# lovelyqian/Embodied-One-Shot-Video-Recognition

Hardware: AMD Instinct MI355X
Metric: clips/sec/GPU (224², 8-seg) + 5-way-1-shot episode acc vs reference (higher is better)
Workload: dtype f32

## Files before the change

embodied-one-shot-video-recognition_amd/csrc/conv_wino_f32.hip:

```cpp
#include <type_traits>

#include "common.h"

namespace eosv {

typedef float f32x4 __attribute__((ext_vector_type(4)));
typedef float f32x16 __attribute__((ext_vector_type(16)));
typedef unsigned u32x4 __attribute__((ext_vector_type(4)));

namespace {
constexpr int WT = 64;
constexpr int WC = 64;
constexpr int WK = 8;
constexpr int IMG = 16 * WK * 64;
constexpr unsigned OOB = 0xffffff00u;
}

template <bool WIDE>
__global__ __launch_bounds__(512) void conv_wino_f32_kernel(WinoArgs a) {
  __shared__ __attribute__((aligned(16))) float smem[5 * IMG];

  const int tid = threadIdx.x;
  const int lane = tid & 63;
  const int wid = __builtin_amdgcn_readfirstlane(tid >> 6);
  const int H = a.H, W = a.W, C = a.C;
  const int TH = (H + 1) >> 1, TW = (W + 1) >> 1, TT = TH * TW;
  const long long T = (long long)a.N * TT;
  const int ncb = C / WC;
  const int nmt = (int)((T + WT - 1) / WT);
  const int nb = nmt * ncb, G = gridDim.x;
  const float* __restrict__ x = a.x;

  auto tile_of = [&](long long t, int& n, int& th, int& tw) {
    int rem;
    if (WIDE) {
      n = (int)(t / TT);
      rem = (int)(t - (long long)n * TT);
    } else {
      n = wino_fdiv((int)t, a.dtt);
      rem = (int)t - n * TT;
    }
    th = wino_fdiv(rem, a.dtw);
    tw = rem - th * TW;
  };

  const int lt = tid >> 3, lc = tid & 7;
  struct Item {
    __amdgpu_buffer_rsrc_t xr;
    unsigned xoff;
    unsigned mask;
    int mt, cb;
  };
  auto decode = [&](int w, int tid) {
    const int lt = tid >> 3, lc = tid & 7;
    Item it;
    const int bt = xcd_tile(w, nb, a.xcd);
    if (a.cbmajor) {
      it.cb = wino_fdiv(bt, a.dnmt);
      it.mt = bt - it.cb * nmt;
    } else {
      it.mt = wino_fdiv(bt, a.dncb);
      it.cb = bt - it.mt * ncb;
    }
    const long long t0 = (long long)it.mt * WT;
    int n0, th, tw;
    tile_of(t0, n0, th, tw);
    const long long xrem = ((long long)a.N - n0) * H * W * C * 4;
    it.xr = __builtin_amdgcn_make_buffer_rsrc((void*)(x + (long long)n0 * H * W * C), (short)0,
                                              (int)(xrem > OOB ? OOB : xrem), 0x00020000);
    it.xoff = 0;
    it.mask = 0;
    const long long t = t0 + lt;
    if (t < T) {
      int n;
      tile_of(t, n, th, tw);
      const int ih0 = 2 * th - 1, iw0 = 2 * tw - 1;
      it.xoff = (unsigned)(((((long long)(n - n0) * H + ih0) * W + iw0) * C + lc) * 4);
#pragma unroll
      for (int p = 0; p < 4; ++p)
#pragma unroll
        for (int q = 0; q < 4; ++q)
          if ((unsigned)(ih0 + p) < (unsigned)H && (unsigned)(iw0 + q) < (unsigned)W) it.mask |= 1u << (4 * p + q);
    }
    return it;
  };
  const int vrot = (lt + 4 * lc) & 63;
  float d[2][16], t[16];
  __amdgpu_buffer_rsrc_t ld_xr;
  unsigned ld_off[16];
  auto set_taps = [&](const Item& it) {
    ld_xr = it.xr;
#pragma unroll
    for (int p = 0; p < 4; ++p)
#pragma unroll
      for (int q = 0; q < 4; ++q) {
        const bool in = (it.mask >> (4 * p + q)) & 1;
        ld_off[4 * p + q] = in ? it.xoff + (unsigned)((p * W + q) * C * 4) : OOB;
      }
  };
  auto load_rows = [&](float* ds, int kc, int p0) {
#pragma unroll
    for (int i = 4 * p0; i < 4 * p0 + 8; ++i)
      ds[i] = __builtin_bit_cast(float, __builtin_amdgcn_raw_buffer_load_b32(ld_xr, (int)ld_off[i], kc * (WK * 4), 0));
  };
  auto row_stage = [&](float* ds) {
#pragma unroll
    for (int i = 0; i < 16; ++i) asm volatile("" : "+v"(ds[i]));
#pragma unroll
    for (int q = 0; q < 4; ++q) {
      const float* z = ds + q;
      t[q] = z[0] - z[8];
      t[4 + q] = z[4] + z[8];
      t[8 + q] = z[8] - z[4];
      t[12 + q] = z[4] - z[12];
    }
  };
  auto store_row = [&](float* Vs, int p) {
    float* dst = Vs + lc * 64 + vrot;
    dst[(4 * p + 0) * (WK * 64)] = t[4 * p] - t[4 * p + 2];
    dst[(4 * p + 1) * (WK * 64)] = t[4 * p + 1] + t[4 * p + 2];
    dst[(4 * p + 2) * (WK * 64)] = t[4 * p + 2] - t[4 * p + 1];
    dst[(4 * p + 3) * (WK * 64)] = t[4 * p + 1] - t[4 * p + 3];
  };
  const unsigned ulane = (wid * 4) * 256 + lane * 4;
  auto dma_u = [&](int cb, int kc, float* Us) {
    const float* us = a.u + ((long long)cb * (C / WK) + kc) * IMG;
#pragma unroll
    for (int j = 0; j < 4; ++j)
      __builtin_amdgcn_global_load_lds((const void*)(us + (ulane + j * 256)),
                                       (__attribute__((address_space(3))) void*)(Us + (wid * 4 + j) * 256), 16, 0, 0);
  };
  auto sync_ring = [&](auto ahead) {
    vm_wait<decltype(ahead)::value>();
    asm volatile("s_waitcnt lgkmcnt(0)" ::: "memory");
    __builtin_amdgcn_s_barrier();
    asm volatile("" ::: "memory");
  };
  using std::integral_constant;

  f32x16 acc[2][2][2];

  const int h = lane >> 5, r = lane & 31;
  const int nk = C / WK;
  int w = blockIdx.x;
  Item cur = decode(w, tid);
  Item nxt = decode(w + G < nb ? w + G : w, tid);
  set_taps(cur);
  load_rows(d[0], 0, 0);
  load_rows(d[0], 0, 2);
  dma_u(cur.cb, 0, smem + 2 * IMG);
  row_stage(d[0]);
  load_rows(d[1], 1, 0);
  load_rows(d[1], 1, 2);
  load_rows(d[0], 2, 0);
  load_rows(d[0], 2, 2);
  vm_wait<0>();

  auto chunk = [&](int kc, auto par) {
    constexpr int slot = decltype(par)::value;
    float* dn = d[1 - slot];
    const bool s1 = kc + 1 >= nk, s3 = kc + 3 >= nk;
    const int k1 = s1 ? kc + 1 - nk : kc + 1, k3 = s3 ? kc + 3 - nk : kc + 3;
    const int cb1 = s1 ? nxt.cb : cur.cb;
    float* Un = smem + (3 - slot) * IMG;
    const float* Vs = smem + slot * IMG + (2 * wid) * (WK * 64);
    const float* Us = smem + (2 + slot) * IMG + (2 * wid) * (WK * 64);
    float* Vn = smem + (1 - slot) * IMG;
    float a0[2], a1[2], b0[2], b1[2];
    auto read_ops = [&](int g) {
      const int k = 2 * (g & 3) + h;
      const float* vr = Vs + (g >> 2) * (WK * 64) + k * 64;
      const float* ur = Us + (g >> 2) * (WK * 64) + k * 64;
      a0[g & 1] = vr[(r + 4 * k) & 63];
      a1[g & 1] = vr[(r + 32 + 4 * k) & 63];
      b0[g & 1] = ur[r];
      b1[g & 1] = ur[32 + r];
    };
    read_ops(0);
#pragma unroll
    for (int g = 0; g < 8; ++g) {
      if (g < 7) read_ops(g + 1);
      if (g == 0) row_stage(dn);
      if (g == 1) {
        if (slot == 1 && kc + 3 == nk) set_taps(nxt);
        dma_u(cb1, k1, Un);
        __builtin_amdgcn_sched_barrier(0);
      }
      if (g == 1 || g == 2) load_rows(dn, k3, 2 * (g - 1));
      if (g >= 3 && g < 7) store_row(Vn, g - 3);
      const int p = g >> 2, c = g & 1;
      acc[p][0][0] = __builtin_amdgcn_mfma_f32_32x32x2f32(a0[c], b0[c], acc[p][0][0], 0, 0, 0);
      acc[p][0][1] = __builtin_amdgcn_mfma_f32_32x32x2f32(a0[c], b1[c], acc[p][0][1], 0, 0, 0);
      acc[p][1][0] = __builtin_amdgcn_mfma_f32_32x32x2f32(a1[c], b0[c], acc[p][1][0], 0, 0, 0);
      acc[p][1][1] = __builtin_amdgcn_mfma_f32_32x32x2f32(a1[c], b1[c], acc[p][1][1], 0, 0, 0);
      __builtin_amdgcn_sched_barrier(0);
    }
    sync_ring(integral_constant<int, 16>{});
  };

  float* __restrict__ y = a.y;
  const float* __restrict__ res = a.res;
  for (;;) {
#pragma unroll
    for (int p = 0; p < 4; ++p) store_row(smem, p);
    {
      Item c = cur;
      asm volatile("" : "+v"(c.xoff), "+v"(c.mask));
      set_taps(c);
    }
#pragma unroll
    for (int p = 0; p < 2; ++p)
#pragma unroll
      for (int i = 0; i < 2; ++i)
#pragma unroll
        for (int j = 0; j < 2; ++j)
#pragma unroll
          for (int q = 0; q < 16; ++q) acc[p][i][j][q] = 0.f;
    asm volatile("s_waitcnt lgkmcnt(0)" ::: "memory");
    __builtin_amdgcn_s_barrier();
    asm volatile("" ::: "memory");
    for (int kc = 0; kc < nk; kc += 2) {
      chunk(kc, integral_constant<int, 0>{});
      chunk(kc + 1, integral_constant<int, 1>{});
    }

    int te;
    asm volatile("v_mbcnt_lo_u32_b32 %0, -1, 0\n\tv_mbcnt_hi_u32_b32 %0, -1, %0" : "=v"(te));
    te += wid * 64;
    const int trow = te >> 4, c4 = te & 15, he = (te >> 5) & 1, re = te & 31;
    const int we = __builtin_amdgcn_readfirstlane(te >> 6);
    const int mup = we >= 4 ? IMG : 0;
    const int mt = cur.mt;
    const int co = cur.cb * WC + c4 * 4;
    w += G;
    const bool more = w < nb;
    cur = nxt;
    f32x4 bv = {0.f, 0.f, 0.f, 0.f};
    if (a.bias) bv = *(const f32x4*)(a.bias + co);
    int n0, th0, tw0;
    tile_of((long long)mt * WT, n0, th0, tw0);
    const long long fbytes = (long long)H * W * C * 4, yrem = ((long long)a.N - n0) * fbytes;
    const int yrec = (int)(yrem > OOB ? OOB : yrem);
    const __amdgpu_buffer_rsrc_t yr =
        __builtin_amdgcn_make_buffer_rsrc((void*)((char*)y + n0 * fbytes), (short)0, yrec, 0x00020000);
    const __amdgpu_buffer_rsrc_t rr = __builtin_amdgcn_make_buffer_rsrc(
        (void*)(res ? (const char*)res + n0 * fbytes : (const char*)nullptr), (short)0, res ? yrec : 0, 0x00020000);
#pragma unroll
    for (int i = 0; i < 2; ++i) {
      if (i) __syncthreads();
#pragma unroll
      for (int p = 0; p < 2; ++p)
#pragma unroll
        for (int j = 0; j < 2; ++j)
#pragma unroll
          for (int q = 0; q < 16; ++q)
            smem[(2 * we + p) * (32 * WC) + mup + ((q & 3) + 8 * (q >> 2) + 4 * he) * WC + j * 32 + re] = acc[p][i][j][q];
      __builtin_amdgcn_sched_barrier(0);
      const long long tl = (long long)mt * WT + i * 32 + trow;
      unsigned o[4];
      f32x4 rv[4];
      {
        int n, th, tw;
        tile_of(tl < T ? tl : 0, n, th, tw);
#pragma unroll
        for (int e = 0; e < 4; ++e) {
          const int oh = 2 * th + (e >> 1), ow = 2 * tw + (e & 1);
          const bool ok = tl < T && oh < H && ow < W;
          o[e] = ok ? (unsigned)(((((long long)(n - n0) * H + oh) * W + ow) * C + co) * 4) : OOB;
          rv[e] = __builtin_bit_cast(f32x4, __builtin_amdgcn_raw_buffer_load_b128(rr, (int)o[e], 0, 0));
        }
      }
      if (i == 1) nxt = decode(w + G < nb ? w + G : w < nb ? w : w - G, te);
      __syncthreads();
      f32x4 s[8];
#pragma unroll
      for (int q = 0; q < 4; ++q) {
        f32x4 m[4];
#pragma unroll
        for (int p = 0; p < 4; ++p)
          m[p] = *(const f32x4*)(smem + (4 * p + q) * (32 * WC) + (p >= 2 ? IMG : 0) + trow * WC + c4 * 4);
        s[q] = (m[0] + m[1]) + m[2];
        s[4 + q] = (m[1] - m[2]) - m[3];
        if (q & 1) __builtin_amdgcn_sched_barrier(0);
      }
      if (i) {
        __syncthreads();
        __builtin_amdgcn_sched_barrier(0);
      }
#pragma unroll
      for (int e = 0; e < 4; ++e) {
        const int dy = e >> 1;
        f32x4 v = (e & 1) ? (s[4 * dy + 1] - s[4 * dy + 2]) - s[4 * dy + 3] : (s[4 * dy] + s[4 * dy + 1]) + s[4 * dy + 2];
        v += bv;
        if (res) v += rv[e];
        if (a.relu) {
          v.x = fmaxf(v.x, 0.f);
          v.y = fmaxf(v.y, 0.f);
          v.z = fmaxf(v.z, 0.f);
          v.w = fmaxf(v.w, 0.f);
        }
        __builtin_amdgcn_raw_buffer_store_b128(__builtin_bit_cast(u32x4, v), yr, (int)o[e], 0, 0);
      }
    }
    if (!more) break;
  }
  vm_wait<0>();
}

bool conv_wino_f32_ok(int C) { return C >= WC && C % WC == 0; }

int launch_conv_wino_f32(const WinoArgs& a0, hipStream_t s) {
  if (!conv_wino_f32_ok(a0.C) || a0.N <= 0 || a0.H <= 0 || a0.W <= 0)
    return set_error("conv_wino_f32: needs C % 64 == 0 and a non-empty input"), EOSV_ERR_UNSUPPORTED;
  const long long T = (long long)a0.N * ((a0.H + 1) / 2) * ((a0.W + 1) / 2);
  const long long nb = ((T + WT - 1) / WT) * (a0.C / WC);
  if (nb > 0x7fffffffLL) return set_error("conv_wino_f32: grid too large"), EOSV_ERR_UNSUPPORTED;
  if (65LL * a0.H * a0.W * a0.C * 4 > 0xffffffffLL)
    return set_error("conv_wino_f32: 65 frames exceed 32-bit byte offsets"), EOSV_ERR_UNSUPPORTED;
  if (a0.plan) return record_launch(a0.plan, nb, 1);
  WinoArgs a = a0;
  a.cbmajor = a.C >= 512;
  const int TW = (a.W + 1) / 2, TT = ((a.H + 1) / 2) * TW;
  a.dtt = wino_div(TT);
  a.dtw = wino_div(TW);
  a.dncb = wino_div(a.C / WC);
  a.dnmt = wino_div((unsigned)((T + WT - 1) / WT));
  const bool wide = T + 2 * WT > 0x7fffffffLL;
  const long long G = std::min<long long>(nb, a.max_wg > 0 ? a.max_wg : device_cu_count());
  if (wide)
    hipLaunchKernelGGL(conv_wino_f32_kernel<true>, dim3((unsigned)G), dim3(512), 0, s, a);
  else
    hipLaunchKernelGGL(conv_wino_f32_kernel<false>, dim3((unsigned)G), dim3(512), 0, s, a);
  EOSV_LAUNCH_CHECK();
  return EOSV_OK;
}

namespace {
constexpr int GROW = 65;
constexpr int GTAP = 8 * GROW;
}

__global__ __launch_bounds__(512) void wino_weights_kernel(const float* __restrict__ w, int cin, int nchunk, int flip,
                                                           float* __restrict__ u) {
  __shared__ float gs[9 * GTAP];
  const int tid = threadIdx.x;
  const int ob = blockIdx.x / nchunk, kc = blockIdx.x - ob * nchunk;
  const int o0 = ob * 64, i0 = kc * 8;
#pragma unroll
  for (int j = 0; j < 9; ++j) {
    const int e = j * 512 + tid;
    if (flip) {
      const int o = e & 63, r = e >> 6;
      const int i = r / 9, tap = r - 9 * i;
      gs[(8 - tap) * GTAP + i * GROW + o] = w[((size_t)i0 * 9 + r) * cin + o0 + o];
    } else {
      const int i = e & 7, r = e >> 3;
      const int o = r / 9, tap = r - 9 * o;
      gs[tap * GTAP + i * GROW + o] = w[((size_t)o0 * 9 + r) * cin + i0 + i];
    }
  }
  __syncthreads();
  const int i = tid >> 6, o = tid & 63;
  double gf[9];
#pragma unroll
  for (int k = 0; k < 9; ++k) gf[k] = (double)gs[k * GTAP + i * GROW + o];
  constexpr double G[4][3] = {{1, 0, 0}, {0.5, 0.5, 0.5}, {0.5, -0.5, 0.5}, {0, 0, 1}};
  double Gg[4][3];
#pragma unroll
  for (int p = 0; p < 4; ++p)
#pragma unroll
    for (int c = 0; c < 3; ++c) Gg[p][c] = G[p][0] * gf[c] + G[p][1] * gf[3 + c] + G[p][2] * gf[6 + c];
  float* dst = u + (size_t)blockIdx.x * IMG + i * 64 + o;
#pragma unroll
  for (int p = 0; p < 4; ++p)
#pragma unroll
    for (int q = 0; q < 4; ++q)
      dst[(4 * p + q) * (WK * 64)] = (float)(Gg[p][0] * G[q][0] + Gg[p][1] * G[q][1] + Gg[p][2] * G[q][2]);
}

}

extern "C" int eosv_wino_weights_f32(const float* w_ocihw, const float* alpha_or_null, int cout, int cin,
                                     float* u_out) {
  using namespace eosv;
  if (!w_ocihw || !u_out || cout <= 0 || cin <= 0 || cout % 64 || cin % 8)
    return set_error("eosv_wino_weights_f32: needs cout % 64 == 0 and cin % 8 == 0"), EOSV_ERR_ARG;
  static const double G[4][3] = {{1, 0, 0}, {0.5, 0.5, 0.5}, {0.5, -0.5, 0.5}, {0, 0, 1}};
  for (int o = 0; o < cout; ++o) {
    const float al = alpha_or_null ? alpha_or_null[o] : 1.f;
    for (int i = 0; i < cin; ++i) {
      const float* g = w_ocihw + ((size_t)o * cin + i) * 9;
      float gf[9];
      for (int k = 0; k < 9; ++k) gf[k] = alpha_or_null ? g[k] * al : g[k];
      double Gg[4][3];
      for (int p = 0; p < 4; ++p)
        for (int c = 0; c < 3; ++c) Gg[p][c] = G[p][0] * gf[c] + G[p][1] * gf[3 + c] + G[p][2] * gf[6 + c];
      for (int p = 0; p < 4; ++p)
        for (int q = 0; q < 4; ++q)
          u_out[wino_u_index(o, i, 4 * p + q, cin)] =
              (float)(Gg[p][0] * G[q][0] + Gg[p][1] * G[q][1] + Gg[p][2] * G[q][2]);
    }
  }
  return EOSV_OK;
}

extern "C" int eosv_wino_weights_f32_device(const float* d_w_ohwi, int cout, int cin, int flip, float* d_u,
                                            eosv_stream_t stream) {
  using namespace eosv;
  if (!d_w_ohwi || !d_u) return set_error("eosv_wino_weights_f32_device: null pointer"), EOSV_ERR_ARG;
  if (flip != 0 && flip != 1) return set_error("eosv_wino_weights_f32_device: flip must be 0 or 1"), EOSV_ERR_ARG;
  const int oc = flip ? cin : cout, ic = flip ? cout : cin;
  if (cout <= 0 || cin <= 0 || oc % 64 || ic % 8)
    return set_error(flip ? "eosv_wino_weights_f32_device: flip = 1 needs cin % 64 == 0 and cout % 8 == 0"
                          : "eosv_wino_weights_f32_device: flip = 0 needs cout % 64 == 0 and cin % 8 == 0"),
           EOSV_ERR_ARG;
  const long long nb = (long long)(oc / 64) * (ic / 8);
  if (nb > 0x7fffffffLL) return set_error("eosv_wino_weights_f32_device: grid too large"), EOSV_ERR_ARG;
  hipLaunchKernelGGL(wino_weights_kernel, dim3((unsigned)nb), dim3(512), 0, (hipStream_t)stream, d_w_ohwi, cin,
                     ic / 8, flip, d_u);
  EOSV_LAUNCH_CHECK();
  return EOSV_OK;
}

namespace eosv {
static int conv_wino_f32_entry(const float* d_x, const float* d_u, const float* d_bias, const float* d_res, int relu,
                               float* d_y, int N, int H, int W, int C, int max_wg, eosv_stream_t stream) {
  if (!d_x || !d_u || !d_y || N <= 0 || H <= 0 || W <= 0 || C <= 0)
    return set_error("eosv_conv_wino_f32: bad argument"), EOSV_ERR_ARG;
  WinoArgs a{};
  a.max_wg = max_wg;
  a.x = d_x;
  a.u = d_u;
  a.bias = d_bias;
  a.res = d_res;
  a.y = d_y;
  a.N = N;
  a.H = H;
  a.W = W;
  a.C = C;
  a.relu = relu;
  a.xcd = 1;
  return launch_conv_wino_f32(a, (hipStream_t)stream);
}
}

extern "C" int eosv_conv_wino_f32(const float* d_x, const float* d_u, const float* d_bias, const float* d_res,
                                  int relu, float* d_y, int N, int H, int W, int C, eosv_stream_t stream) {
  return eosv::conv_wino_f32_entry(d_x, d_u, d_bias, d_res, relu, d_y, N, H, W, C, 0, stream);
}

extern "C" int eosv_conv_wino_f32_grid(const float* d_x, const float* d_u, const float* d_bias, const float* d_res,
                                       int relu, float* d_y, int N, int H, int W, int C, eosv_stream_t stream,
                                       int max_workgroups) {
  if (max_workgroups <= 0)
    return eosv::set_error("eosv_conv_wino_f32_grid: max_workgroups must be positive"), EOSV_ERR_ARG;
  return eosv::conv_wino_f32_entry(d_x, d_u, d_bias, d_res, relu, d_y, N, H, W, C, max_workgroups, stream);
}
```

Baseline: 3385.

## Vectorize Winograd V-operand LDS reads and interleave DMA/loads with MFMA scheduling

Changes the LDS layout of the transformed input tile so each lane's A-operand values for four k-steps are contiguous, replacing scalar LDS reads with one 128-bit read per half-tile. It also splits the U-tile DMA and input-row loads into per-step pieces spread across the eight MFMA groups, and adds sched_group_barrier hints to interleave MFMA with the other instructions. The aim is fewer LDS instructions and smoother overlap of memory traffic with matrix math. Risks include LDS bank conflicts from the new layout, higher register pressure from the vector operands, and a rigid schedule that may stall.

```diff
diff --git a/embodied-one-shot-video-recognition_amd/csrc/conv_wino_f32.hip b/embodied-one-shot-video-recognition_amd/csrc/conv_wino_f32.hip
--- a/embodied-one-shot-video-recognition_amd/csrc/conv_wino_f32.hip
+++ b/embodied-one-shot-video-recognition_amd/csrc/conv_wino_f32.hip
@@ -84,7 +84,7 @@
     }
     return it;
   };
-  const int vrot = (lt + 4 * lc) & 63;
+  const int vword = (lc & 1) * 256 + ((lt + 4 * (lc & 1)) & 63) * 4 + (lc >> 1);
   float d[2][16], t[16];
   __amdgpu_buffer_rsrc_t ld_xr;
   unsigned ld_off[16];
@@ -98,9 +98,9 @@
         ld_off[4 * p + q] = in ? it.xoff + (unsigned)((p * W + q) * C * 4) : OOB;
       }
   };
-  auto load_rows = [&](float* ds, int kc, int p0) {
-#pragma unroll
-    for (int i = 4 * p0; i < 4 * p0 + 8; ++i)
+  auto load_row = [&](float* ds, int kc, int p) {
+#pragma unroll
+    for (int i = 4 * p; i < 4 * p + 4; ++i)
       ds[i] = __builtin_bit_cast(float, __builtin_amdgcn_raw_buffer_load_b32(ld_xr, (int)ld_off[i], kc * (WK * 4), 0));
   };
   auto row_stage = [&](float* ds) {
@@ -116,19 +116,25 @@
     }
   };
   auto store_row = [&](float* Vs, int p) {
-    float* dst = Vs + lc * 64 + vrot;
+    float* dst = Vs + vword;
     dst[(4 * p + 0) * (WK * 64)] = t[4 * p] - t[4 * p + 2];
     dst[(4 * p + 1) * (WK * 64)] = t[4 * p + 1] + t[4 * p + 2];
     dst[(4 * p + 2) * (WK * 64)] = t[4 * p + 2] - t[4 * p + 1];
     dst[(4 * p + 3) * (WK * 64)] = t[4 * p + 1] - t[4 * p + 3];
   };
   const unsigned ulane = (wid * 4) * 256 + lane * 4;
+  auto dma_piece = [&](int cb, int kc, float* Us, int j) {
+    const float* us = a.u + ((long long)cb * (C / WK) + kc) * IMG;
+    __builtin_amdgcn_global_load_lds((const void*)(us + (ulane + j * 256)),
+                                     (__attribute__((address_space(3))) void*)(Us + (wid * 4 + j) * 256), 16, 0, 0);
+  };
   auto dma_u = [&](int cb, int kc, float* Us) {
-    const float* us = a.u + ((long long)cb * (C / WK) + kc) * IMG;
-#pragma unroll
-    for (int j = 0; j < 4; ++j)
-      __builtin_amdgcn_global_load_lds((const void*)(us + (ulane + j * 256)),
-                                       (__attribute__((address_space(3))) void*)(Us + (wid * 4 + j) * 256), 16, 0, 0);
+#pragma unroll
+    for (int j = 0; j < 4; ++j) dma_piece(cb, kc, Us, j);
+  };
+  auto load_patch = [&](float* ds, int kc) {
+#pragma unroll
+    for (int p = 0; p < 4; ++p) load_row(ds, kc, p);
   };
   auto sync_ring = [&](auto ahead) {
     vm_wait<decltype(ahead)::value>();
@@ -141,19 +147,17 @@
   f32x16 acc[2][2][2];
 
   const int h = lane >> 5, r = lane & 31;
+  const int va0 = h * 256 + (r + 4 * h) * 4, va1 = h * 256 + ((r + 32 + 4 * h) & 63) * 4;
   const int nk = C / WK;
   int w = blockIdx.x;
   Item cur = decode(w, tid);
   Item nxt = decode(w + G < nb ? w + G : w, tid);
   set_taps(cur);
-  load_rows(d[0], 0, 0);
-  load_rows(d[0], 0, 2);
+  load_patch(d[0], 0);
   dma_u(cur.cb, 0, smem + 2 * IMG);
   row_stage(d[0]);
-  load_rows(d[1], 1, 0);
-  load_rows(d[1], 1, 2);
-  load_rows(d[0], 2, 0);
-  load_rows(d[0], 2, 2);
+  load_patch(d[1], 1);
+  load_patch(d[0], 2);
   vm_wait<0>();
 
   auto chunk = [&](int kc, auto par) {
@@ -166,33 +170,43 @@
     const float* Vs = smem + slot * IMG + (2 * wid) * (WK * 64);
     const float* Us = smem + (2 + slot) * IMG + (2 * wid) * (WK * 64);
     float* Vn = smem + (1 - slot) * IMG;
-    float a0[2], a1[2], b0[2], b1[2];
-    auto read_ops = [&](int g) {
-      const int k = 2 * (g & 3) + h;
-      const float* vr = Vs + (g >> 2) * (WK * 64) + k * 64;
-      const float* ur = Us + (g >> 2) * (WK * 64) + k * 64;
-      a0[g & 1] = vr[(r + 4 * k) & 63];
-      a1[g & 1] = vr[(r + 32 + 4 * k) & 63];
+    f32x4 a0[2], a1[2];
+    float b0[2], b1[2];
+    auto read_a = [&](int p) {
+      a0[p] = *(const f32x4*)(Vs + p * (WK * 64) + va0);
+      a1[p] = *(const f32x4*)(Vs + p * (WK * 64) + va1);
+    };
+    auto read_b = [&](int g) {
+      const float* ur = Us + (g >> 2) * (WK * 64) + (2 * (g & 3) + h) * 64;
       b0[g & 1] = ur[r];
       b1[g & 1] = ur[32 + r];
     };
-    read_ops(0);
+    read_a(0);
+    read_b(0);
 #pragma unroll
     for (int g = 0; g < 8; ++g) {
-      if (g < 7) read_ops(g + 1);
+      if (g < 7) read_b(g + 1);
+      if (g == 2) read_a(1);
       if (g == 0) row_stage(dn);
-      if (g == 1) {
-        if (slot == 1 && kc + 3 == nk) set_taps(nxt);
-        dma_u(cb1, k1, Un);
-        __builtin_amdgcn_sched_barrier(0);
-      }
-      if (g == 1 || g == 2) load_rows(dn, k3, 2 * (g - 1));
-      if (g >= 3 && g < 7) store_row(Vn, g - 3);
-      const int p = g >> 2, c = g & 1;
-      acc[p][0][0] = __builtin_amdgcn_mfma_f32_32x32x2f32(a0[c], b0[c], acc[p][0][0], 0, 0, 0);
-      acc[p][0][1] = __builtin_amdgcn_mfma_f32_32x32x2f32(a0[c], b1[c], acc[p][0][1], 0, 0, 0);
-      acc[p][1][0] = __builtin_amdgcn_mfma_f32_32x32x2f32(a1[c], b0[c], acc[p][1][0], 0, 0, 0);
-      acc[p][1][1] = __builtin_amdgcn_mfma_f32_32x32x2f32(a1[c], b1[c], acc[p][1][1], 0, 0, 0);
+      if (g >= 1 && g < 5) store_row(Vn, g - 1);
+      if (g < 4) {
+        dma_piece(cb1, k1, Un, g);
+      } else {
+        if (g == 4 && slot == 1 && kc + 3 == nk) set_taps(nxt);
+        load_row(dn, k3, g - 4);
+      }
+      const int p = g >> 2, kp = g & 3, c = g & 1;
+      acc[p][0][0] = __builtin_amdgcn_mfma_f32_32x32x2f32(a0[p][kp], b0[c], acc[p][0][0], 0, 0, 0);
+      acc[p][0][1] = __builtin_amdgcn_mfma_f32_32x32x2f32(a0[p][kp], b1[c], acc[p][0][1], 0, 0, 0);
+      acc[p][1][0] = __builtin_amdgcn_mfma_f32_32x32x2f32(a1[p][kp], b0[c], acc[p][1][0], 0, 0, 0);
+      acc[p][1][1] = __builtin_amdgcn_mfma_f32_32x32x2f32(a1[p][kp], b1[c], acc[p][1][1], 0, 0, 0);
+#pragma unroll
+      for (int i = 0; i < 4; ++i) {
+        __builtin_amdgcn_sched_group_barrier(0x008, 1, 0);
+        if (g == 0) __builtin_amdgcn_sched_group_barrier(0x096, 10, 0);
+        if (g >= 1 && g < 5) __builtin_amdgcn_sched_group_barrier(0x096, 3, 0);
+        if (g >= 5) __builtin_amdgcn_sched_group_barrier(0x096, 2, 0);
+      }
       __builtin_amdgcn_sched_barrier(0);
     }
     sync_ring(integral_constant<int, 16>{});
```

Measured after the change: 3634 (median of 6 runs). 7.3% higher.
